# tub-rip/emba

Measured on AMD Instinct MI355X. Metric: events/sec through warp+Jacobian+JtJ build, 1M events, 1024x2048 pano, higher is better.
Workload: dtype f64; 1 GPU; synthetic N=1000000 sensor=240x180 pano=1024x2048 K=21 seed=20240907; events_per_gpu=1000000, total_events=1000000, thres_valid_pixel=5, cost=quadratic, parallelism=single GPU, events_per_rank=1000000, ep_in_step=True, inliers_rank0=675197, candidates_rank0=956800, active_pixels=68600

## Files before the change

emba_amd/csrc/context.h:

```cpp
#pragma once
#include "../../include/emba_hip.h"

#include <hip/hip_runtime.h>

#include <algorithm>
#include <cmath>
#include <cstdarg>
#include <cstdio>
#include <string>
#include <vector>

#include "kernels.h"
#include "solve_kernels.h"
#include "map_rule.h"
#include "cmax_rule.h"

struct DevBuf {
    void* p = nullptr;
    size_t bytes = 0;
    DevBuf() = default;
    DevBuf(DevBuf&& o) noexcept : p(o.p), bytes(o.bytes) { o.p = nullptr; o.bytes = 0; }
    DevBuf& operator=(DevBuf&& o) noexcept { if (this != &o) { reset(); std::swap(p, o.p); std::swap(bytes, o.bytes); } return *this; }
    ~DevBuf() { reset(); }
    template <typename T> T* as() const { return static_cast<T*>(p); }
// ... 94 lines not shown
    const uint8_t* global_u8 = nullptr;
    double fused_alpha = 0.0;
};

struct WindowState {
    bool have_events = false;
    size_t n_in = 0, n_used = 0, n_halo = 0, n_pm = 0, n_sorted = 0, n_batch = 0, n_cand = 0;
    long nblk = 0;
    long n_fblk = 0, n_fsup = 0;
    size_t P_prev = 0;
    size_t n_outside_tile = 0; int n_rebin = 0; uint32_t last_rebin_stamp = 0;
};

struct OrderState {
    bool keys_ready = false; int64_t key_t0 = 0, key_dt = 0; int key_K = 0;
    uint32_t* d_ev_pix = nullptr; uint32_t* d_ev_batch = nullptr;
    bool tile_order = false, have_ev_pm = false;
    long n_chunks = 0;
    size_t n_lead = 0;
    bool chunks_lpt = false;
    int tile_shape = 0; bool tile_fine = false;
    double order_per_px = 0.0, order_lead_frac = 0.0;
    double order_inl_pred = 0.0;
};

enum StatusWord : int {
    kStFirstBad = 0,
    kStUnsorted = 1,
    kStProbeA = 0, kStProbeB = 1,
    kStBadHalo = 2,
    kStTotal = 4,
    kStHeads = 6,
    kStCounter = 8,
    kStatusWords = 16
};

struct ListsKey {
    bool packed = false; uint32_t stamp = 0; size_t P = 0, nrec = 0; long lo = 0;
    bool operator==(const ListsKey& o) const { return packed == o.packed && stamp == o.stamp && P == o.P && nrec == o.nrec && lo == o.lo; }
};

struct SolveCache {
    bool lists_valid = false; ListsKey key;
    bool perm_valid = false;
    size_t perm_lo = 0, perm_n = 0;
    size_t x2_resident_P = (size_t)-1;
// ... 56 lines not shown
    bool spun = false;
    int* h_pinned_dev = nullptr;
    double* h_knots_dev = nullptr;

    WindowState win;
    OrderState order;
    DevBuf d_pm_pix, d_pm_batch, d_pm_orig;
    DevBuf d_ev_slot;
    DevBuf d_ev_pix_own, d_ev_batch_own;
    DevBuf d_ev_pm;
    DevBuf d_cp, d_batch_u;
    DevBuf d_ev_u, d_ev_seg;
    DevBuf d_chunks;
    int segpose_mode = 0;
    int order_mode = 0;
    DevBuf d_batch_t, d_pose;
    DevBuf d_seg;
    int step_gather = 2;
    DevBuf d_seg_act;
    PostWarpState post;
    int step_one_set = 1;
    int step_fast = 1;
    int use_tags = 1;
    DevBuf d_slot_key; uint32_t rec_stamp = 0;
    RecordSet work, alt;
    bool eq_in_alt = false;
    EqState eq, eq_saved;
    EvalState ev;
    DevBuf d_e_sorted, d_flag, d_inl_idx;
    int opt_poison = 0;
    int opt_tile_reserve = 2, opt_tile_shape = -1, opt_tile_fine = -1, opt_tile_min_events = 1650000, opt_tile_chunk = 0;
    int opt_gather_waves = 0, opt_chunk_order_bin = 0, opt_solve_counts = -1, opt_syrk_dense = 0, opt_syrk_lists = 0, opt_gram_sparse = -1, opt_gram_sparse_chunk = 4, opt_syrk_min_cols = 512, opt_syrk_item_cap = 4096, opt_solve_debug = 0, opt_poisson = 0, opt_gemm64 = 0;
    int step_ep = 1;
    DevBuf d_fblk_cnt, d_fblk_off;
    DevBuf d_fsup;
    DevBuf d_ep;
    double set_events_ms = 0, prepare_ms = 0;

    size_t n_inliers = 0;
    int cost_irls = 0; double cost_eta = 0.0;
    double* h_knots = nullptr; int h_knots_cap = 0; hipEvent_t knots_copied = nullptr; bool knots_in_flight = false;

    hipEvent_t ev_start[8]{}, ev_stop[8]{};
    bool kernel_timing = false;
    hipEvent_t kt_sets[16][5]{}; hipEvent_t* kt = kt_sets[0]; int kt_slot = 0;
    bool kt_valid[16][3]{};
    bool kt_all = false;
    hipEvent_t cal_ev[2]{};
    DevBuf d_probe;
    bool kt_warp_valid = false, kt_accum_valid = false;
    int n_cu = 256;
    int ablate = 0;
    struct {
        DevBuf scan_sums, scan_offs;
        DevBuf sort_hist;
// ... 87 lines not shown
```

emba_amd/csrc/emba_hip.hip:

```cpp
#include "../../include/emba_hip.h"

#include <hip/hip_runtime.h>

#include <algorithm>
#include <atomic>
#include <cmath>
#include <cstdarg>
#include <cstdio>
#include <cstdlib>
#include <cstring>
#include <limits>
#include <string>
#include <vector>

#include "kernels.h"
#include "order_kernels.h"
#include "solve_kernels.h"
#include "poisson_kernels.h"
#include "render_kernels.h"
#include "sequence_kernels.h"
#include "context.h"
#include "sequence_rule.h"

using namespace emba;
// ... 457 lines not shown
    {"tile_reserve", &emba_ctx::opt_tile_reserve, 0, 5},
    {"tile_shape", &emba_ctx::opt_tile_shape, -1, kNumTileShapes - 1},
    {"tile_fine", &emba_ctx::opt_tile_fine, -1, 1},
    {"tile_min_events", &emba_ctx::opt_tile_min_events, 0, 2000000000},
    {"tile_chunk", &emba_ctx::opt_tile_chunk, 0, 1 << 20},
    {"solve_counts", &emba_ctx::opt_solve_counts, -1, 2},
    {"syrk_dense", &emba_ctx::opt_syrk_dense, 0, 1},
    {"syrk_lists", &emba_ctx::opt_syrk_lists, 0, 2},
    {"gram_sparse", &emba_ctx::opt_gram_sparse, -1, 1},
    {"gram_sparse_chunk", &emba_ctx::opt_gram_sparse_chunk, 1, 8},
    {"syrk_min_cols", &emba_ctx::opt_syrk_min_cols, 64, 4096},
    {"syrk_item_cap", &emba_ctx::opt_syrk_item_cap, 1, 65536},
    {"solve_debug", &emba_ctx::opt_solve_debug, 0, 1},
    {"poisson", &emba_ctx::opt_poisson, 0, 2},
    {"gemm64", &emba_ctx::opt_gemm64, 0, 1},
};
const OptionRef kStepPrepOptions[] = {
    {"step_prep", &emba_ctx::step_prep, 0, 1},
    {"step_prep_polls", &emba_ctx::step_prep_polls, 0, 1 << 16},
};
const OptionRef kContrastOptions[] = {
    {"contrast_vote", &emba_ctx::opt_contrast_vote, -1, 1},
};
}

emba_status emba_set_option(emba_ctx* c, const char* name, int32_t value)
{
    if (!c || !name) return EMBA_ERR_INVALID_ARG;
    for (const OptionRef& o : kOptions)
        if (!strcmp(o.name, name)) {
            if (value < o.lo || value > o.hi) return fail(c, EMBA_ERR_INVALID_ARG, "option %s: %d outside [%d, %d]", name, (int)value, o.lo, o.hi);
            c->*(o.field) = (int)value;
            if (!strcmp(name, "order") || !strcmp(name, "chunk_order_bin") || !strncmp(name, "tile_", 5)) c->order.keys_ready = false;
            return EMBA_OK;
        }
    for (const OptionRef& o : kStepPrepOptions)
        if (!strcmp(o.name, name)) {
            if (value < o.lo || value > o.hi) return fail(c, EMBA_ERR_INVALID_ARG, "option %s: %d outside [%d, %d]", name, (int)value, o.lo, o.hi);
            c->*(o.field) = (int)value;
            return EMBA_OK;
        }
    for (const OptionRef& o : kContrastOptions)
        if (!strcmp(o.name, name)) {
            if (value < o.lo || value > o.hi) return fail(c, EMBA_ERR_INVALID_ARG, "option %s: %d outside [%d, %d]", name, (int)value, o.lo, o.hi);
            c->*(o.field) = (int)value;
            return EMBA_OK;
        }
    return fail(c, EMBA_ERR_INVALID_ARG, "unknown option '%s'", name);
}

emba_status emba_get_option(emba_ctx* c, const char* name, int32_t* value)
{
    if (!c || !name || !value) return EMBA_ERR_INVALID_ARG;
    if (!strcmp(name, "prep_in_warp")) { *value = c->ev.prep_in_warp ? 1 : 0; return EMBA_OK; }
    if (!strcmp(name, "texels_packed")) { *value = c->ev.texels_packed ? 1 : 0; return EMBA_OK; }
    if (!strcmp(name, "step_prep_fallbacks")) {
        unsigned n = 0;
        HIP_TRY(c, hipSetDevice(c->device));
        HIP_TRY(c, hipStreamSynchronize(c->stream));
        c->spun = false; c->knots_in_flight = false;
        HIP_TRY(c, hipMemcpy(&n, c->d_seg_flag.as<unsigned>() + 32, sizeof n, hipMemcpyDeviceToHost));
        *value = (int32_t)std::min<unsigned>(n, 0x7FFFFFFFu);
        return EMBA_OK;
    }
    if (!strcmp(name, "ep_valid")) { *value = c->ev.ep_valid ? 1 : 0; return EMBA_OK; }
    for (const OptionRef& o : kOptions)
        if (!strcmp(o.name, name)) { *value = c->*(o.field); return EMBA_OK; }
    for (const OptionRef& o : kStepPrepOptions)
        if (!strcmp(o.name, name)) { *value = c->*(o.field); return EMBA_OK; }
    if (!strcmp(name, "contrast_vote_path")) { *value = c->contrast_vote_path; return EMBA_OK; }
    for (const OptionRef& o : kContrastOptions)
        if (!strcmp(o.name, name)) { *value = c->*(o.field); return EMBA_OK; }
    return fail(c, EMBA_ERR_INVALID_ARG, "unknown option '%s'", name);
}

emba_status emba_last_counts(emba_ctx* c, size_t* n_inliers, size_t* P)
{
    if (!c) return EMBA_ERR_INVALID_ARG;
    HIP_TRY(c, hipSetDevice(c->device));
    emba_status st = resolve_pending(c, true);
    if (st) return st;
    if (n_inliers) *n_inliers = c->n_inliers;
    if (P) *P = c->eq.P;
    return EMBA_OK;
}

emba_status emba_sync(emba_ctx* c)
{
    if (!c) return EMBA_ERR_INVALID_ARG;
    HIP_TRY(c, hipSetDevice(c->device));
    emba_status st = resolve_pending(c);
    if (st) return st;
    HIP_TRY(c, hipStreamSynchronize(c->stream));
    c->spun = false;
// ... 352 lines not shown
```

emba_amd/csrc/kernels.h:

```cpp
#pragma once
#include <hip/hip_runtime.h>
#include <stdint.h>

#include "device_math.h"
#include "order_rule.h"
#include "step_rule.h"

#ifdef EMBA_DIAG
#define EMBA_ABL(word, bit) (((word) & (bit)) != 0)
#else
#define EMBA_ABL(word, bit) false
#endif

namespace emba {

constexpr uint32_t kNoSlot = 0xFFFFFFFFu;
constexpr uint32_t kInvalidPix = 0xFFFFFFFFu;

__device__ __forceinline__ bool record_valid(double tail_y, uint32_t stamp, uint32_t& pano_idx)
{
    pano_idx = (uint32_t)__double2loint(tail_y);
    return (uint32_t)__double2hiint(tail_y) == stamp && pano_idx != kInvalidPix;
}
__host__ __device__ __forceinline__ int32_t count_marker(uint32_t stamp) { return (int32_t)(0x80000000u | (stamp & 0x3FFFFFFFu)); }
// ... 1397 lines not shown
            const int i = b * 64 + threadIdx.x;
            if (p.seg) seg_thread(i, knots, p.K, p.seg);
            else pose_thread(i, p.batch_t_ns, p.nb, knots, p.K, p.t0_ns, p.dt_ns, p.pose, p.err);
        }
    } else if (b < p.n_pose + p.n_tex) {
        texel_rect_blocks((long)b - p.n_pose, p.n_tex, p.Gx, p.Gy, p.H, p.W, p.rect, p.texel);
    } else {
        prep_block(b - p.n_pose - p.n_tex, p.count, p.npix, p.pixacc);
    }
}

typedef double double4_t __attribute__((ext_vector_type(4)));

struct GramParams {
    const double* rec; const uint32_t* slot_key; long n_slots; int chunk;
    const uint32_t* active_bits; int irls; double eta;
    uint32_t stamp;
    const double* tag;
    double* A11; double* b1; int dim;
    int ablate;
    int gather_waves;
    int n_gram_blocks;
    const uint8_t* ep_flag; const double* ep_e; double* ep_out; const uint32_t* ep_fblk_cnt; long ep_n_pm, ep_n_fblk; const uint32_t* ep_fsup;
};

__device__ __forceinline__ void gram_atomic_out(double v, int row, int col, uint32_t key, double* A11, double* b1, int dim, int ablate)
{
    if (row >= 12 || v == 0.0 || EMBA_ABL(ablate, 32)) return;
    const int bc = 3 * (int)(key >> 16), bp = 3 * (int)(key & 0xFFFFu);
    const int grow = (row < 6) ? bc + row : bp + row - 6;
    if (col < 12) {
        const int gcol = (col < 6) ? bc + col : bp + col - 6;
        atomicAdd(A11 + (size_t)grow + (size_t)dim * gcol, v);
    } else if (col == 14) {
        atomicAdd(b1 + grow, v);
    }
}

typedef __attribute__((address_space(3))) uint32_t lds_u32_t;
typedef __attribute__((address_space(3))) double lds_f64_t;
__device__ __attribute__((noinline)) void gram_flush(double4_t ee, double4_t oe, double4_t oo, uint32_t key, double* A11, double* b1,
                                                     uint32_t dim_ablate, uint32_t lds_tag_tile)
{
    const int dim = (int)(dim_ablate & 0x3FFFFu), ablate = (int)(dim_ablate >> 18);
    uint32_t* const s_tag = (uint32_t*)(lds_u32_t*)(uintptr_t)((lds_tag_tile & 0xFFFFu) << 2);
    double* const s_tile = (double*)(lds_f64_t*)(uintptr_t)((lds_tag_tile >> 16) << 3);
// ... 39 lines not shown
            const int i = q + 4 * r;
            tile[(2 * i) * 16 + 2 * j] = e;
            tile[(2 * i + 1) * 16 + 2 * j] = x;
            tile[(2 * j) * 16 + 2 * i + 1] = x;
            tile[(2 * i + 1) * 16 + 2 * j + 1] = o;
        }
    }
}

__device__ __forceinline__ double rec_elem14(double2 v)
{
    return __hiloint2double(__builtin_amdgcn_ds_swizzle(__double2hiint(v.x), (7 << 5) | 0x18),
                            __builtin_amdgcn_ds_swizzle(__double2loint(v.x), (7 << 5) | 0x18));
}
__device__ __forceinline__ uint32_t rec_elem15_lo(double2 v)
{
    return (uint32_t)__builtin_amdgcn_ds_swizzle(__double2loint(v.y), (7 << 5) | 0x18);
}
__device__ __forceinline__ uint32_t rec_elem15_hi(double2 v)
{
    return (uint32_t)__builtin_amdgcn_ds_swizzle(__double2hiint(v.y), (7 << 5) | 0x18);
}

template <bool TAGS, int kGramBlock, bool GATHER, bool SPARSE = false>
__device__ __forceinline__ void gram_body(const GramParams& p, const long gram_blk, const ActiveWriteParams& aw)
{
    __shared__ uint32_t s_tag[kGramKeys];
    __shared__ double s_tile[kGramKeys * 256];
    __shared__ uint32_t s_pre[GATHER ? kGatherMaxUnits + 1 : 1];
    __shared__ uint32_t s_ws[kGramBlock / 64];
    __shared__ double s_wtile[(kGramBlock / 64) * 256];
    __shared__ uint32_t s_wkey[kGramBlock / 64];
    for (int i = threadIdx.x; i < kGramKeys * 256; i += kGramBlock) s_tile[i] = 0.0;
    if (threadIdx.x < kGramKeys) s_tag[threadIdx.x] = 0xFFFFFFFFu;
    if (threadIdx.x < kGramBlock / 64) s_wkey[threadIdx.x] = 0xFFFFFFFFu;
    const int kGW = GATHER ? __builtin_amdgcn_readfirstlane(p.gather_waves) : 0, kSW = kGramBlock / 64 - kGW;
    if (GATHER) {
        const uint32_t P_act = active_gather_prefix<kGramBlock>(aw, gram_blk, s_pre, s_ws);
        if (threadIdx.x < 64 * kGW) {
            if (kGW == 1) active_gather_slice<64>(aw, gram_blk, p.n_gram_blocks, P_act, s_pre);
            else if (kGW == 2) active_gather_slice<128>(aw, gram_blk, p.n_gram_blocks, P_act, s_pre);
            else active_gather_slice<256>(aw, gram_blk, p.n_gram_blocks, P_act, s_pre);
        }
    } else {
        __syncthreads();
    }
    const int lane = threadIdx.x & 63;
    const int wv = __builtin_amdgcn_readfirstlane(threadIdx.x >> 6) - kGW;
    constexpr int U = TAGS ? GRAM_U : GRAM_U_NT;
    constexpr int TS = GRAM_SPARSE_TS;
    constexpr int kStage = SPARSE ? 64 * TS : 8 * U;
    const int kStride = kSW * kStage;
    const long start = gram_blk * (kGramBlock / 64) * p.chunk;
    const long end = (start + (long)(kGramBlock / 64) * p.chunk < p.n_slots) ? start + (long)(kGramBlock / 64) * p.chunk : p.n_slots;
    const int len = (int)(end - start);
    const int off0 = wv * kStage;
    const bool have_work = wv >= 0 && off0 < len;
    const int m = lane & 7, R = lane >> 3;
    if (have_work) {

    uint32_t cur_key = p.slot_key[start + off0];
    bool dirty = false;
    double4_t acc_ee = {0.0, 0.0, 0.0, 0.0}, acc_oe = acc_ee, acc_oo = acc_ee;
    auto flush = [&]() {
        gram_flush(acc_ee, acc_oe, acc_oo, cur_key, p.A11, p.b1, (uint32_t)p.dim | ((uint32_t)p.ablate << 18),
                   (((uint32_t)(uintptr_t)(lds_u32_t*)s_tag >> 2) & 0xFFFFu) | (((uint32_t)(uintptr_t)(lds_f64_t*)s_tile >> 3) << 16));
#pragma unroll
        for (int r = 0; r < 4; ++r) { acc_ee[r] = 0.0; acc_oe[r] = 0.0; acc_oo[r] = 0.0; }
    };
    double2 xA[U], xB[U];
    uint32_t act[U], k_first = 0, k_last = 0;
    const double2* rec0 = reinterpret_cast<const double2*>(p.rec + (size_t)kRecStride * start) + lane;
    const uint32_t* key0 = p.slot_key + start;
    auto load_records = [&](int off, double2* x) {
        const double2* q = rec0 + 8 * off;
#pragma unroll
        for (int u = 0; u < U; ++u) {
            typedef double v2d __attribute__((ext_vector_type(2)));
            if (GRAM_NT_LOAD) { const v2d v = __builtin_nontemporal_load(reinterpret_cast<const v2d*>(q + 64 * u)); x[u] = make_double2(v.x, v.y); }
// ... 1 lines not shown
        }
    };
    auto lookup = [&](int off, const double2* x) {
        k_first = key0[off];
        k_last = key0[(off + 8 * U < len ? off + 8 * U : len) - 1];
#pragma unroll
        for (int u = 0; u < U; ++u) {
            const uint32_t pi = rec_elem15_lo(x[u]);
            const bool in = off + 8 * u + R < len;
            const bool valid = in && rec_elem15_hi(x[u]) == p.stamp && pi != kInvalidPix;
            act[u] = valid ? (EMBA_ABL(p.ablate, 256) ? ~0u : p.active_bits[pi >> 5]) >> (pi & 31) : 0u;
        }
    };
    auto weight = [&](const double2& x) {
        double w = 1.0;
        if (p.irls) {
            const double e = rec_elem14(x);
            if (p.irls == 2) w = 1.0 / (1.0 + p.eta * e * e);
            else { const double a = fabs(e); w = (a < p.eta) ? 1.0 : p.eta / a; }
        }
        return w;
    };
    auto consume = [&](int off, double2* x) {
        if ((k_first == cur_key) && (k_last == cur_key)) {
#pragma unroll
            for (int u = 0; u < U; ++u) {
                const bool ok = act[u] & 1u;
                const double w = weight(x[u]);
                const double ax = ok ? w * x[u].x : 0.0, ay = ok ? w * x[u].y : 0.0, bx = ok ? x[u].x : 0.0, by = ok ? x[u].y : 0.0;
                if (__ballot(ok)) {
                    dirty = true;
                    if (!EMBA_ABL(p.ablate, 64)) {
                        acc_ee = __builtin_amdgcn_mfma_f64_16x16x4f64(ax, bx, acc_ee, 0, 0, 0);
                        acc_oe = __builtin_amdgcn_mfma_f64_16x16x4f64(ay, bx, acc_oe, 0, 0, 0);
                        acc_oo = __builtin_amdgcn_mfma_f64_16x16x4f64(ay, by, acc_oo, 0, 0, 0);
                    }
                }
            }
            return;
        }
        double2* y = x;
        uint32_t* a_ = act;
#pragma unroll 1
        for (int u = 0; u < U; ++u) {
            const bool ok = a_[0] & 1u;
            const double w = weight(y[0]);
            const int s = off + 8 * u + R;
// ... 151 lines not shown
            const uint32_t bit = ((EMBA_ABL(p.ablate, 256) ? ~0u : w) >> ((uint32_t)__double2loint(tg) & 31u)) & (tagvalid(off, tg) ? 1u : 0u);
            return (unsigned long long)__ballot(bit != 0);
        };
        const double2* dummy = reinterpret_cast<const double2*>(p.rec + (size_t)kRecStride * start) + (lane & 7);
        auto load_masked = [&](int off, unsigned long long m, double2* x) {
            const double2* q = rec0 + 8 * off;
#pragma unroll
            for (int u = 0; u < U; ++u) {
#if GRAM_DUMMY_LOADS
                x[u] = *(((m >> (8 * u + R)) & 1u) ? q + 64 * u : dummy);
#else
                if (GRAM_TAG_NT) {
                    typedef double v2d __attribute__((ext_vector_type(2)));
                    v2d v = {0.0, 0.0};
                    if ((m >> (8 * u + R)) & 1u) v = __builtin_nontemporal_load(reinterpret_cast<const v2d*>(q + 64 * u));
                    x[u] = make_double2(v.x, v.y);
                } else
                x[u] = ((m >> (8 * u + R)) & 1u) ? q[64 * u] : make_double2(0.0, 0.0);
#endif
            }
        };
        typedef const uint32_t __attribute__((address_space(4))) * const_u32_ptr;
        const_u32_ptr key_s = (const_u32_ptr)(uintptr_t)key0;
        auto keys = [&](int off) { k_first = key_s[off]; k_last = key_s[(off + 8 * U < len ? off + 8 * U : len) - 1]; };
        static_assert(8 * U <= 64, "a stage's live mask is one wave ballot");
        unsigned long long Mc; uint32_t W;
        double Te, To;
        auto iterate = [&](int off, double2* cur, double2* nxt, double& Tb, double& Tn) {
            const bool h1 = off + kStride < len;
            const unsigned long long Mn = h1 ? bitmask(off + kStride, Tb, W) : 0ull;
            W = bitword(off + 2 * kStride, Tn);
            Tb = tagload(off + 3 * kStride);
            load_masked(h1 ? off + kStride : off, Mn, nxt);
            keys(off);
#pragma unroll
            for (int u = 0; u < U; ++u) act[u] = (Mc >> (8 * u + R)) & 1u;
            if (Mc) consume(off, cur);
            Mc = Mn;
        };
        Te = tagload(off0);
        W = bitword(off0, Te);
        To = tagload(off0 + kStride);
        Mc = bitmask(off0, Te, W);
        W = bitword(off0 + kStride, To);
        Te = tagload(off0 + 2 * kStride);
        load_masked(off0, Mc, xA);
        for (int off = off0; off < len;) {
// ... 37 lines not shown
    uint32_t actA[U];
    load_clamped(off0, xA);
    load_clamped(off0 + kStride, xB);
    load_clamped(off0 + 2 * kStride, xC);
    lookup_into(off0, xA, actA, kfA, klA);
    for (int off = off0; off < len;) {
        iterate(off, xA, xB, xD, actA, kfA, klA, actB, kfB, klB); off += kStride; if (off >= len) break;
        iterate(off, xB, xC, xA, actB, kfB, klB, actA, kfA, klA); off += kStride; if (off >= len) break;
        iterate(off, xC, xD, xB, actA, kfA, klA, actB, kfB, klB); off += kStride; if (off >= len) break;
        iterate(off, xD, xA, xC, actB, kfB, klB, actA, kfA, klA); off += kStride;
    }
    }
#if !GRAM_WAVE_TILE
    if (dirty) flush();
#else
    if (dirty) {
        const int wabs = threadIdx.x >> 6;
        gram_wave_tile(acc_ee, acc_oe, acc_oo, s_wtile + wabs * 256);
        if (lane == 0) s_wkey[wabs] = cur_key;
    }
#endif
    }
    __syncthreads();
    for (int i = threadIdx.x; i < kGramKeys * 256; i += kGramBlock) {
        const uint32_t key = s_tag[i >> 8];
        if (key != 0xFFFFFFFFu) gram_atomic_out(s_tile[i], (i >> 4) & 15, i & 15, key, p.A11, p.b1, p.dim, p.ablate);
    }
    if (threadIdx.x < 256) {
        const int e = threadIdx.x, row = e >> 4, col = e & 15;
        constexpr int NW = kGramBlock / 64;
        uint32_t kw[NW];
#pragma unroll
        for (int w = 0; w < NW; ++w) kw[w] = s_wkey[w];
        double tv[NW];
#pragma unroll
        for (int w = 0; w < NW; ++w) tv[w] = (kw[w] != 0xFFFFFFFFu) ? s_wtile[w * 256 + e] : 0.0;
        if (row < 12 && (col < 12 || col == 14)) {
#pragma unroll
            for (int w = 0; w < NW; ++w) {
                if (kw[w] == 0xFFFFFFFFu) continue;
                bool leader = true;
#pragma unroll
                for (int w2 = 0; w2 < w; ++w2) leader = leader && (kw[w2] != kw[w]);
                if (!leader) continue;
                double sum = 0.0;
#pragma unroll
// ... 26 lines not shown
        const double2 a = *reinterpret_cast<const double2*>(p.ep_e + i0), b = *reinterpret_cast<const double2*>(p.ep_e + i0 + 2);
        e[0] = a.x; e[1] = a.y; e[2] = b.x; e[3] = b.y;
    } else {
#pragma unroll
        for (int k = 0; k < 4; ++k) if (i0 + k < p.ep_n_pm) { fl |= (uint32_t)p.ep_flag[i0 + k] << (8 * k); e[k] = p.ep_e[i0 + k]; }
    }
    const uint32_t m = ((fl & 0xFFu) ? 1u : 0u) | ((fl & 0xFF00u) ? 2u : 0u) | ((fl & 0xFF0000u) ? 4u : 0u) | ((fl & 0xFF000000u) ? 8u : 0u);
    const uint32_t mine = __popc(m);
    uint32_t x = mine;
#pragma unroll
    for (int o = 1; o < 64; o <<= 1) { const uint32_t y = __shfl_up(x, o); if (lane >= o) x += y; }
#pragma unroll
    for (int o = 32; o >= 1; o >>= 1) part += __shfl_xor(part, o);
    if (lane == 63) s_x[wv] = x;
    if (lane == 0) s_b[wv] = part;
    __syncthreads();
    uint32_t k = x - mine;
#pragma unroll
    for (int w = 0; w < kGramBlock / 64; ++w) { k += s_b[w]; if (w < wv) k += s_x[w]; }
#pragma unroll
    for (int q = 0; q < 4; ++q) if (m & (1u << q)) p.ep_out[k++] = e[q];
}

template <bool TAGS, bool GATHER, bool SPARSE = false>
__global__ __launch_bounds__(kGramBlock) void emba_gram_kernel(GramParams p, ActiveWriteParams aw)
{
    if ((int)blockIdx.x >= p.n_gram_blocks) { ep_tail_block((long)blockIdx.x - p.n_gram_blocks, p); return; }
    gram_body<TAGS, kGramBlock, GATHER, SPARSE>(p, blockIdx.x, aw);
}

__global__ void emba_a22_from_records_kernel(const double* __restrict__ rec, long n_slots, const int32_t* __restrict__ count,
                                             const int32_t* __restrict__ compact, int thres, int irls, double eta,
                                             double* __restrict__ A22b2, uint32_t stamp)
{
    const long s = (long)blockIdx.x * blockDim.x + threadIdx.x;
    if (s >= n_slots) return;
    const double2* r2 = reinterpret_cast<const double2*>(rec + (size_t)kRecStride * s);
    const double2 tail = r2[7];
    uint32_t pi;
    if (!record_valid(tail.y, stamp, pi) || count[pi] < thres) return;
    const double e = tail.x;
    double w = 1.0;
    if (irls == 2) w = 1.0 / (1.0 + eta * e * e);
    else if (irls == 1) { const double a = fabs(e); w = (a < eta) ? 1.0 : eta / a; }
    const double ew = w * e;
    const double2 d = r2[6];
    double* q = A22b2 + 5 * (size_t)compact[pi];
    atomicAdd(q + 0, w * (d.x * d.x));
    atomicAdd(q + 1, w * (d.x * d.y));
    atomicAdd(q + 2, w * (d.y * d.y));
    atomicAdd(q + 3, d.x * ew);
// ... 206 lines not shown
```

emba_amd/csrc/order_host.h:

```cpp
#pragma once
#include "context.h"
#include "order_kernels.h"
#include "sequence_rule.h"

#include <chrono>

using namespace emba;

namespace {

OrderState new_order(const OrderState& prev)
{
    OrderState o{};
    o.tile_shape = prev.tile_shape; o.tile_fine = prev.tile_fine;
    return o;
}
void free_window(emba_ctx* c)
{
    WindowState w{};
    w.last_rebin_stamp = c->rec_stamp - 3;
    w.n_rebin = c->win.n_rebin;
    w.n_used = c->win.n_used; w.n_cand = c->win.n_cand; w.n_sorted = c->win.n_sorted; w.n_outside_tile = c->win.n_outside_tile;
    c->win = w;
    OrderState o = new_order(c->order);
// ... 254 lines not shown
emba_status assign_record_slots(emba_ctx* c, int K)
{
    hipStream_t s = c->stream;
    emba_status st;
    const size_t nd = c->win.n_sorted, M = c->win.n_cand;
    if ((st = ensure<uint32_t>(c, c->ord.pos, std::max<size_t>(nd, 1)))) return st;
    uint32_t *d_cf = c->ord.flags.as<uint32_t>(), *d_cpos = c->ord.pos.as<uint32_t>();
    if ((st = dev_scan(c, d_cf, d_cpos, nd, nullptr))) return st;
    if ((st = ensure_sort_pairs(c, std::max<size_t>(M, 1)))) return st;
    uint32_t *k0 = c->ord.keys[0].as<uint32_t>(), *v0 = c->ord.vals[0].as<uint32_t>(), *k1 = c->ord.keys[1].as<uint32_t>(), *v1 = c->ord.vals[1].as<uint32_t>();
    if ((st = ensure<uint32_t>(c, c->d_ev_slot, nd))) return st;
    HIP_TRY(c, hipMemsetAsync(c->d_ev_slot.as<uint32_t>(), 0xFF, std::max<size_t>(nd, 1) * 4, s));
    if (nd) hipLaunchKernelGGL(emba_cand_keys_kernel, dim3(nblocks(nd)), dim3(256), 0, s, c->order.d_ev_pix, c->order.d_ev_batch, c->d_cp.as<uint16_t>(), (long)nd, d_cpos, k0, v0);
    const int kb = bits_for((size_t)K);
    if (kb <= 8) {
        if (M) hipLaunchKernelGGL(emba_fold_keys_kernel, dim3(nblocks(M)), dim3(256), 0, s, k0, (long)M, 1);
        if ((st = dev_sort(c, &k0, &v0, &k1, &v1, M, 16))) return st;
        if (M) hipLaunchKernelGGL(emba_fold_keys_kernel, dim3(nblocks(M)), dim3(256), 0, s, k0, (long)M, 0);
    } else if ((st = dev_sort(c, &k0, &v0, &k1, &v1, M, 32))) return st;
    if (M) hipLaunchKernelGGL(emba_slot_assign_kernel, dim3(nblocks(M)), dim3(256), 0, s, k0, v0, (long)M, c->d_ev_slot.as<uint32_t>(), c->d_slot_key.as<uint32_t>());
    return EMBA_OK;
}

emba_status prepare_order(emba_ctx* c, const double* knots_host, int64_t t0, int64_t dt, int K)
{
    if (c->order.keys_ready && c->order.key_t0 == t0 && c->order.key_dt == dt && c->order.key_K == K) return EMBA_OK;
    if (dt <= 0 || K < 2 || K > 65535) return fail(c, EMBA_ERR_INVALID_ARG, "bad spline: dt_ns=%lld K=%d", (long long)dt, K);
    const auto t_begin = std::chrono::steady_clock::now();
    hipStream_t s = c->stream;
    emba_status st;
    const size_t ns = c->win.n_pm;
    c->order = new_order(c->order);
    TileOrderChoice choice;
    if ((st = order_batch_segments(c, t0, dt, K)) || (st = choose_tile_order(c, knots_host, t0, dt, K, &choice))) return st;
    if ((st = choice.tile ? build_tile_order(c, choice) : build_pixel_order(c))) return st;
    c->win.nblk = (long)((c->win.n_sorted + kWarpNew - 1) / kWarpNew);
    if ((st = assign_record_slots(c, K))) return st;
    if ((st = ensure<double>(c, c->d_e_sorted, ns)) || (st = ensure<uint8_t>(c, c->d_flag, ns)) || (st = ensure<int32_t>(c, c->d_inl_idx, ns))) return st;
    HIP_TRY(c, hipMemsetAsync(c->d_flag.as<uint8_t>(), 0, std::max<size_t>(ns, 1), s));
    HIP_TRY(c, hipGetLastError());
    HIP_TRY(c, hipStreamSynchronize(s));
    c->order.keys_ready = true; c->order.key_t0 = t0; c->order.key_dt = dt; c->order.key_K = K;
    c->prepare_ms = std::chrono::duration<double, std::milli>(std::chrono::steady_clock::now() - t_begin).count();
    return EMBA_OK;
}


emba_status size_record_set(emba_ctx* c, RecordSet& rs, size_t n_cand)
{
    bool rec_fresh = false, tag_fresh = false;
    emba_status st;
    if ((st = ensure<double>(c, rs.rec, (std::max<size_t>(n_cand, 1) + kGramPad) * kRecStride, &rec_fresh)) || (st = ensure<double>(c, rs.tag, n_cand + kGramPad, &tag_fresh)))
        return st;
    if (rec_fresh) HIP_TRY(c, hipMemsetAsync(rs.rec.p, 0, rs.rec.bytes, c->stream));
    if (tag_fresh) HIP_TRY(c, hipMemsetAsync(rs.tag.p, 0, rs.tag.bytes, c->stream));
    return EMBA_OK;
}

emba_status set_events_core(emba_ctx* c, const uint16_t* x, const uint16_t* y, const uint8_t* pol, const int64_t* t_dev, const int64_t* batch_t_host,
                            size_t n, const uint16_t* hx, const uint16_t* hy, const int64_t* hbt, size_t n_halo)
// ... 172 lines not shown
```

emba_amd/csrc/order_kernels.h:

```cpp
#pragma once
#include <hip/hip_runtime.h>
#include <stdint.h>

#include "device_math.h"
#include "order_rule.h"

namespace emba {

constexpr uint32_t kEvPol = 0x80000000u;
constexpr uint32_t kEvLead = 0x40000000u;
constexpr uint32_t kEvHasPred = 0x20000000u;
constexpr uint32_t kEvPixMask = 0x1FFFFFFFu;
constexpr uint32_t kValHalo = 0x80000000u;
constexpr uint32_t kNoBin = 0xFFFFFFFFu;

constexpr int kSortTile = 4096;
constexpr int kScanTile = 4096;

__global__ __launch_bounds__(256) void emba_scan_tile_sums_kernel(const uint32_t* __restrict__ in, long n, uint32_t* __restrict__ sums)
{
    __shared__ uint32_t s_w[4];
    const long base = (long)blockIdx.x * kScanTile + 16 * threadIdx.x;
    uint32_t acc = 0;
#pragma unroll
// ... 331 lines not shown
__global__ void emba_cand_flag_kernel(const uint32_t* __restrict__ ev_pix, long nd, uint32_t* __restrict__ cand_flag)
{
    const long j = (long)blockIdx.x * blockDim.x + threadIdx.x;
    if (j < nd) cand_flag[j] = (ev_pix[j] & kEvHasPred) ? 1u : 0u;
}

__global__ void emba_fold_keys_kernel(uint32_t* __restrict__ keys, long M, int fold)
{
    const long m = (long)blockIdx.x * blockDim.x + threadIdx.x;
    if (m >= M) return;
    const uint32_t k = keys[m];
    keys[m] = fold ? (((k >> 16) << 8) | (k & 0xFFu)) : (((k >> 8) << 16) | (k & 0xFFu));
}

__global__ void emba_slot_assign_kernel(const uint32_t* __restrict__ keys, const uint32_t* __restrict__ vals, long M, uint32_t* __restrict__ ev_slot,
                                        uint32_t* __restrict__ slot_key)
{
    const long s = (long)blockIdx.x * blockDim.x + threadIdx.x;
    if (s >= M) return;
    ev_slot[vals[s]] = (uint32_t)s;
    slot_key[s] = keys[s];
}

__global__ void emba_fill_u32_kernel(uint32_t* __restrict__ p, long n, uint32_t v)
{
    const long i = (long)blockIdx.x * blockDim.x + threadIdx.x;
    if (i < n) p[i] = v;
}

__global__ void emba_iota_kernel(uint32_t* __restrict__ p, long n)
{
    const long i = (long)blockIdx.x * blockDim.x + threadIdx.x;
    if (i < n) p[i] = (uint32_t)i;
}

__global__ __launch_bounds__(256) void emba_count_pred_inliers_kernel(const uint32_t* __restrict__ pm_pix, const uint32_t* __restrict__ pred, long ns, double outlier_px,
                                                                      unsigned long long* __restrict__ out)
{
    __shared__ uint32_t s_w[4];
    uint32_t acc = 0;
    const double lim2 = outlier_px * outlier_px;
    for (long i = (long)blockIdx.x * 256 + threadIdx.x; i < ns; i += (long)gridDim.x * 256) {
        if (i == 0 || !(pm_pix[i] & kEvHasPred) || (pm_pix[i] & kEvLead)) continue;
        const uint32_t a = pred[i], b = pred[i - 1];
        if (a == kNoPixel || b == kNoPixel) continue;
        const double dx = (double)(int)(a & 0xFFFFu) - (double)(int)(b & 0xFFFFu), dy = (double)(int)(a >> 16) - (double)(int)(b >> 16);
// ... 23 lines not shown
```

emba_amd/csrc/step_host.h:

```cpp
#pragma once
#include "context.h"
#include "step_rule.h"

using namespace emba;

namespace {

#define STEP_TRY(call) do { if (const emba_status st_ = (call)) return st_; } while (0)

constexpr GramSizes kGramSizes{kGramBlock, kGramChunk, kGramChunkMin, kEpTailBlk};

emba_status check_irls(emba_ctx* c, int32_t irls)
{
    if (irls < 0 || irls > 2) return fail(c, EMBA_ERR_INVALID_ARG, "irls must be 0 (quadratic), 1 (huber) or 2 (cauchy)");
    return EMBA_OK;
}

bool gram_uses_tags(const emba_ctx* c, bool ep_host) { return gram_tags(c->use_tags, c->order.tile_order, ep_host); }

emba_status ensure_pack(emba_ctx* c, int K)
{
    const PackLayout pack(K);
    if (c->pack_bound) {
        if (c->pack_cap < pack.head)
// ... 506 lines not shown
namespace {

emba_status override_ep(emba_ctx* c, const double* ep_host)
{
    hipStream_t s = c->stream;
    STEP_TRY(ensure_inl_idx(c));
    HIP_TRY(c, hipMemcpyAsync(c->d_ep.as<double>(), ep_host, c->n_inliers * sizeof(double), hipMemcpyHostToDevice, s));
    hipLaunchKernelGGL(emba_override_ep_kernel, dim3((unsigned)((c->win.n_sorted + 255) / 256)), dim3(256), 0, s, c->d_ep.as<double>(), c->d_flag.as<uint8_t>(),
                       c->d_inl_idx.as<int32_t>(), c->d_ev_slot.as<uint32_t>(), c->order.d_ev_pix, c->order.tile_order ? c->d_ev_pm.as<uint32_t>() : nullptr, (long)c->win.n_sorted, c->work.rec.as<double>(), c->d_e_sorted.as<double>());
    return EMBA_OK;
}

emba_status rebuild_a22_from_records(emba_ctx* c, int32_t irls, double eta)
{
    hipStream_t s = c->stream;
    STEP_TRY(ensure_compact(c));
    HIP_TRY(c, hipMemsetAsync(pack_A22b2(c), 0, 5 * c->eq.P * sizeof(double), s));
    if (c->win.n_cand)
        hipLaunchKernelGGL(emba_a22_from_records_kernel, dim3((unsigned)((c->win.n_cand + 255) / 256)), dim3(256), 0, s, c->work.rec.as<double>(),
                           (long)c->win.n_cand, c->d_count, c->d_compact.as<int32_t>(), c->eq.thres, irls, eta, pack_A22b2(c), c->work.stamp);
    return EMBA_OK;
}

void launch_gram_form(bool tags, bool gather, bool sparse, unsigned grid, hipStream_t s, const GramParams& p, const ActiveWriteParams& aw)
{
#define GRAM_FORM(...) hipLaunchKernelGGL((emba_gram_kernel<__VA_ARGS__>), dim3(grid), dim3(kGramBlock), 0, s, p, aw)
    if (tags && sparse) { if (gather) GRAM_FORM(true, true, true); else GRAM_FORM(true, false, true); }
    else if (tags) { if (gather) GRAM_FORM(true, true); else GRAM_FORM(true, false); }
    else { if (gather) GRAM_FORM(false, true); else GRAM_FORM(false, false); }
#undef GRAM_FORM
}

emba_status launch_gram(emba_ctx* c, bool ep_host, int32_t irls, double eta)
{
    hipStream_t s = c->stream;
    GramParams p{};
    p.rec = c->work.rec.as<double>(); p.slot_key = c->d_slot_key.as<uint32_t>(); p.n_slots = (long)c->win.n_cand;
    p.active_bits = reinterpret_cast<const uint32_t*>(c->d_active_bits.as<uint8_t>());
    p.irls = irls; p.eta = eta;
    p.stamp = c->work.stamp;
    p.A11 = pack_A11(c); p.b1 = pack_b1(c); p.dim = 3 * c->eq.K;
    p.tag = gram_uses_tags(c, ep_host) ? c->work.tag.as<double>() : nullptr;
    p.ablate = c->ablate;
    const bool sparse = gram_sparse(p.tag != nullptr, c->opt_gram_sparse, c->win.P_prev, c->win.n_cand, c->eq.thres);
    const bool ep_tail = c->ev.ep_in_gram && !ep_host && c->win.n_pm;
    const GramPlan plan = gram_plan(c->win.n_cand, sparse, c->opt_gram_sparse_chunk, c->n_cu, ep_tail, c->win.n_pm, c->opt_gather_waves, kGramSizes);
    p.chunk = plan.chunk;
    p.n_gram_blocks = plan.n_gram_blocks;
    p.gather_waves = plan.gather_waves;
    if (c->kernel_timing) HIP_TRY(c, hipEventRecord(c->kt[2], s));
    if (ep_tail) {
        p.ep_flag = c->d_flag.as<uint8_t>(); p.ep_e = c->d_e_sorted.as<double>(); p.ep_out = c->d_ep.as<double>();
        p.ep_fblk_cnt = c->d_fblk_cnt.as<uint32_t>(); p.ep_n_fblk = c->win.n_fblk;
        p.ep_n_pm = (long)c->win.n_pm;
        p.ep_fsup = c->d_fsup.as<uint32_t>() + (size_t)c->post.fsup_half * c->win.n_fsup * kFlagSupStride;
    }
    c->ev.ep_in_gram = false;
    const ActiveWriteParams aw = c->post.gather_deferred ? c->post.gather : ActiveWriteParams{};
    launch_gram_form(p.tag != nullptr, c->post.gather_deferred, sparse, plan.grid, s, p, aw);
    c->post.gather_deferred = false;
    if (ep_tail) c->ev.ep_valid = true;
    if (c->kernel_timing) { HIP_TRY(c, hipEventRecord(c->kt[3], s)); c->kt_accum_valid = true; c->kt_valid[c->kt_slot][1] = true; }
    return EMBA_OK;
}

emba_status launch_ep_after_gram(emba_ctx* c)
{
    STEP_TRY(dev_scan(c, c->d_fblk_cnt.as<uint32_t>(), c->d_fblk_off.as<uint32_t>(), (size_t)c->win.n_fblk, c->d_total.as<uint32_t>() + 2));
    hipLaunchKernelGGL(emba_compact_ep_kernel, dim3((unsigned)c->win.n_fblk), dim3(256), 0, c->stream, c->d_e_sorted.as<double>(), c->d_flag.as<uint8_t>(), (const uint32_t*)nullptr, c->d_fblk_off.as<uint32_t>(), (long)c->win.n_pm,
                       c->d_ep.as<double>(), (int32_t*)nullptr);
    c->ev.ep_valid = true;
    return EMBA_OK;
}

}

extern "C" emba_status emba_form_accumulate(emba_ctx* c, const double* ep_host, int32_t irls, double eta)
{
    if (!c) return EMBA_ERR_INVALID_ARG;
    if (!c->eq.active_done && !c->ev.P_pending) return fail(c, EMBA_ERR_STATE, "emba_form_active has not been called");
    if (c->eq.accum_done) return fail(c, EMBA_ERR_STATE, "these equations have been accumulated already: A11 | b1 are cleared by emba_form_active only (a second pass would add the sums again)");
    STEP_TRY(check_irls(c, irls));
// ... 131 lines not shown
```

emba_amd/csrc/step_rule.h:

```cpp
#pragma once
#include <stddef.h>
#include <stdint.h>

#include <algorithm>

#if defined(__HIPCC__)
#define EMBA_RULE_HD __host__ __device__
#else
#define EMBA_RULE_HD
#endif

namespace emba {

struct PackLayout {
    size_t b1, A22b2, head;
    explicit PackLayout(int K) : b1((size_t)9 * K * K), A22b2(b1 + (size_t)3 * K), head(A22b2) {}
    size_t len(size_t P) const { return head + 5 * P; }
    size_t need(size_t npix) const { return len(npix); }
    size_t max_P(size_t cap) const { return (cap - head) / 5; }
};

inline int hessian_source(int texel_mode, size_t n_sorted, size_t npix)
{
    return texel_mode == 1 ? 1 : texel_mode == 2 ? 0 : texel_mode == 3 ? 3 : (n_sorted > 4 * npix ? 1 : 3);
}

inline bool segpose_in_pixel_order(bool tile_order, int segpose_mode) { return !tile_order && (segpose_mode ? segpose_mode == 2 : true); }
// ... 46 lines not shown
struct GramPlan { int chunk; long waves; int n_gram_blocks; unsigned ep_tail_blocks, grid; int gather_waves; };
inline GramPlan gram_plan(size_t n_cand, bool sparse, int opt_gram_sparse_chunk, int n_cu, bool ep_tail, size_t n_pm, int opt_gather_waves, const GramSizes& k)
{
    GramPlan g{};
    const long chunk_cap = sparse ? (long)opt_gram_sparse_chunk * k.chunk : k.chunk;
    const long per_round = (long)n_cu * (k.block / 64);
    const long rounds = std::max<long>(1, ((long)n_cand + per_round * chunk_cap - 1) / (per_round * chunk_cap));
    long chunk = ((long)n_cand + per_round * rounds - 1) / (per_round * rounds);
    chunk = (chunk + 7) & ~7L;
    chunk = std::min<long>(std::max<long>(chunk, k.chunk_min), chunk_cap);
    g.chunk = (int)chunk;
    g.waves = ((long)n_cand + chunk - 1) / chunk;
    const long wpb = k.block / 64;
    g.grid = (unsigned)((g.waves + wpb - 1) / wpb);
    g.n_gram_blocks = (int)g.grid;
    if (ep_tail) {
        g.ep_tail_blocks = (unsigned)((n_pm + k.ep_tail_blk - 1) / k.ep_tail_blk);
        g.grid += g.ep_tail_blocks;
    }
    g.gather_waves = gather_waves(opt_gather_waves);
    return g;
}

inline bool tile_rebin_due(bool tile_order, size_t n_inliers, size_t n_outside_tile, uint32_t rec_stamp, uint32_t last_rebin_stamp)
{
    return tile_order && n_inliers && n_outside_tile * 5 > n_inliers && rec_stamp - last_rebin_stamp >= 3;
}

}
```

Measured before the change: 11.19 billion events/s.

## Align gram wave work ranges to single-key runs to skip shared tile merging

Adds a paired gram form. Each wave gets a precomputed [start,end) cut that lies inside one slot-key run, computed on the host from run starts collected after slot assignment. Because every stage then holds a single key, the kernel skips the per-stage key checks, the shared tile zeroing and the final tag-tile atomic flush. The cost is an extra kernel, a host sync and a copy at order preparation, plus possibly more waves and uneven load when runs are short.

```diff
diff --git a/emba_amd/csrc/context.h b/emba_amd/csrc/context.h
--- a/emba_amd/csrc/context.h
+++ b/emba_amd/csrc/context.h
@@ -140,6 +140,8 @@
     int tile_shape = 0; bool tile_fine = false;
     double order_per_px = 0.0, order_lead_frac = 0.0;
     double order_inl_pred = 0.0;
+    std::vector<uint32_t> run_start; bool runs_known = false;
+    int cuts_sw = 0, cuts_base_blocks = 0, cuts_blocks = 0;
 };
 
 enum StatusWord : int {
@@ -242,6 +244,7 @@
     int step_one_set = 1;
     int step_fast = 1;
     int use_tags = 1;
+    DevBuf d_gram_cuts; std::vector<uint32_t> h_gram_cuts; bool last_gram_paired = false;
     DevBuf d_slot_key; uint32_t rec_stamp = 0;
     RecordSet work, alt;
     bool eq_in_alt = false;
@@ -250,7 +253,7 @@
     DevBuf d_e_sorted, d_flag, d_inl_idx;
     int opt_poison = 0;
     int opt_tile_reserve = 2, opt_tile_shape = -1, opt_tile_fine = -1, opt_tile_min_events = 1650000, opt_tile_chunk = 0;
-    int opt_gather_waves = 0, opt_chunk_order_bin = 0, opt_solve_counts = -1, opt_syrk_dense = 0, opt_syrk_lists = 0, opt_gram_sparse = -1, opt_gram_sparse_chunk = 4, opt_syrk_min_cols = 512, opt_syrk_item_cap = 4096, opt_solve_debug = 0, opt_poisson = 0, opt_gemm64 = 0;
+    int opt_gather_waves = 0, opt_chunk_order_bin = 0, opt_solve_counts = -1, opt_syrk_dense = 0, opt_syrk_lists = 0, opt_gram_sparse = -1, opt_gram_sparse_chunk = 4, opt_gram_multikey = 0, opt_syrk_min_cols = 512, opt_syrk_item_cap = 4096, opt_solve_debug = 0, opt_poisson = 0, opt_gemm64 = 0;
     int step_ep = 1;
     DevBuf d_fblk_cnt, d_fblk_off;
     DevBuf d_fsup;
diff --git a/emba_amd/csrc/emba_hip.hip b/emba_amd/csrc/emba_hip.hip
--- a/emba_amd/csrc/emba_hip.hip
+++ b/emba_amd/csrc/emba_hip.hip
@@ -503,6 +503,9 @@
 const OptionRef kContrastOptions[] = {
     {"contrast_vote", &emba_ctx::opt_contrast_vote, -1, 1},
 };
+const OptionRef kGramOptions[] = {
+    {"gram_multikey", &emba_ctx::opt_gram_multikey, 0, 1},
+};
 }
 
 emba_status emba_set_option(emba_ctx* c, const char* name, int32_t value)
@@ -527,6 +530,12 @@
             c->*(o.field) = (int)value;
             return EMBA_OK;
         }
+    for (const OptionRef& o : kGramOptions)
+        if (!strcmp(o.name, name)) {
+            if (value < o.lo || value > o.hi) return fail(c, EMBA_ERR_INVALID_ARG, "option %s: %d outside [%d, %d]", name, (int)value, o.lo, o.hi);
+            c->*(o.field) = (int)value;
+            return EMBA_OK;
+        }
     return fail(c, EMBA_ERR_INVALID_ARG, "unknown option '%s'", name);
 }
 
@@ -551,6 +560,9 @@
         if (!strcmp(o.name, name)) { *value = c->*(o.field); return EMBA_OK; }
     if (!strcmp(name, "contrast_vote_path")) { *value = c->contrast_vote_path; return EMBA_OK; }
     for (const OptionRef& o : kContrastOptions)
+        if (!strcmp(o.name, name)) { *value = c->*(o.field); return EMBA_OK; }
+    if (!strcmp(name, "gram_paired")) { *value = c->last_gram_paired ? 1 : 0; return EMBA_OK; }
+    for (const OptionRef& o : kGramOptions)
         if (!strcmp(o.name, name)) { *value = c->*(o.field); return EMBA_OK; }
     return fail(c, EMBA_ERR_INVALID_ARG, "unknown option '%s'", name);
 }
diff --git a/emba_amd/csrc/kernels.h b/emba_amd/csrc/kernels.h
--- a/emba_amd/csrc/kernels.h
+++ b/emba_amd/csrc/kernels.h
@@ -1443,6 +1443,7 @@
     int gather_waves;
     int n_gram_blocks;
     const uint8_t* ep_flag; const double* ep_e; double* ep_out; const uint32_t* ep_fblk_cnt; long ep_n_pm, ep_n_fblk; const uint32_t* ep_fsup;
+    const uint32_t* wave_cuts;
 };
 
 __device__ __forceinline__ void gram_atomic_out(double v, int row, int col, uint32_t key, double* A11, double* b1, int dim, int ablate)
@@ -1528,7 +1529,7 @@
     return (uint32_t)__builtin_amdgcn_ds_swizzle(__double2hiint(v.y), (7 << 5) | 0x18);
 }
 
-template <bool TAGS, int kGramBlock, bool GATHER, bool SPARSE = false>
+template <bool TAGS, int kGramBlock, bool GATHER, bool SPARSE = false, bool PAIRED = false>
 __device__ __forceinline__ void gram_body(const GramParams& p, const long gram_blk, const ActiveWriteParams& aw)
 {
     __shared__ uint32_t s_tag[kGramKeys];
@@ -1537,8 +1538,11 @@
     __shared__ uint32_t s_ws[kGramBlock / 64];
     __shared__ double s_wtile[(kGramBlock / 64) * 256];
     __shared__ uint32_t s_wkey[kGramBlock / 64];
-    for (int i = threadIdx.x; i < kGramKeys * 256; i += kGramBlock) s_tile[i] = 0.0;
-    if (threadIdx.x < kGramKeys) s_tag[threadIdx.x] = 0xFFFFFFFFu;
+    static_assert(!PAIRED || (TAGS && !SPARSE && GRAM_WAVE_TILE), "the pair-aligned form is the dense tag-stream form with the waves' own tiles");
+    if constexpr (!PAIRED) {
+        for (int i = threadIdx.x; i < kGramKeys * 256; i += kGramBlock) s_tile[i] = 0.0;
+        if (threadIdx.x < kGramKeys) s_tag[threadIdx.x] = 0xFFFFFFFFu;
+    }
     if (threadIdx.x < kGramBlock / 64) s_wkey[threadIdx.x] = 0xFFFFFFFFu;
     const int kGW = GATHER ? __builtin_amdgcn_readfirstlane(p.gather_waves) : 0, kSW = kGramBlock / 64 - kGW;
     if (GATHER) {
@@ -1556,11 +1560,18 @@
     constexpr int U = TAGS ? GRAM_U : GRAM_U_NT;
     constexpr int TS = GRAM_SPARSE_TS;
     constexpr int kStage = SPARSE ? 64 * TS : 8 * U;
-    const int kStride = kSW * kStage;
-    const long start = gram_blk * (kGramBlock / 64) * p.chunk;
-    const long end = (start + (long)(kGramBlock / 64) * p.chunk < p.n_slots) ? start + (long)(kGramBlock / 64) * p.chunk : p.n_slots;
+    const int kStride = PAIRED ? kStage : kSW * kStage;
+    long start, end;
+    if constexpr (PAIRED) {
+        const uint32_t* cut = p.wave_cuts + 2 * (gram_blk * (kGramBlock / 64) + (wv > 0 ? wv : 0));
+        start = (long)__builtin_amdgcn_readfirstlane((int)cut[0]);
+        end = (long)__builtin_amdgcn_readfirstlane((int)cut[1]);
+    } else {
+        start = gram_blk * (kGramBlock / 64) * p.chunk;
+        end = (start + (long)(kGramBlock / 64) * p.chunk < p.n_slots) ? start + (long)(kGramBlock / 64) * p.chunk : p.n_slots;
+    }
     const int len = (int)(end - start);
-    const int off0 = wv * kStage;
+    const int off0 = PAIRED ? 0 : wv * kStage;
     const bool have_work = wv >= 0 && off0 < len;
     const int m = lane & 7, R = lane >> 3;
     if (have_work) {
@@ -1608,7 +1619,7 @@
         return w;
     };
     auto consume = [&](int off, double2* x) {
-        if ((k_first == cur_key) && (k_last == cur_key)) {
+        if (PAIRED || ((k_first == cur_key) && (k_last == cur_key))) {
 #pragma unroll
             for (int u = 0; u < U; ++u) {
                 const bool ok = act[u] & 1u;
@@ -1806,7 +1817,7 @@
         };
         typedef const uint32_t __attribute__((address_space(4))) * const_u32_ptr;
         const_u32_ptr key_s = (const_u32_ptr)(uintptr_t)key0;
-        auto keys = [&](int off) { k_first = key_s[off]; k_last = key_s[(off + 8 * U < len ? off + 8 * U : len) - 1]; };
+        auto keys = [&](int off) { if constexpr (!PAIRED) { k_first = key_s[off]; k_last = key_s[(off + 8 * U < len ? off + 8 * U : len) - 1]; } };
         static_assert(8 * U <= 64, "a stage's live mask is one wave ballot");
         unsigned long long Mc; uint32_t W;
         double Te, To;
@@ -1890,6 +1901,7 @@
 #endif
     }
     __syncthreads();
+    if constexpr (!PAIRED)
     for (int i = threadIdx.x; i < kGramKeys * 256; i += kGramBlock) {
         const uint32_t key = s_tag[i >> 8];
         if (key != 0xFFFFFFFFu) gram_atomic_out(s_tile[i], (i >> 4) & 15, i & 15, key, p.A11, p.b1, p.dim, p.ablate);
@@ -1962,11 +1974,11 @@
     for (int q = 0; q < 4; ++q) if (m & (1u << q)) p.ep_out[k++] = e[q];
 }
 
-template <bool TAGS, bool GATHER, bool SPARSE = false>
+template <bool TAGS, bool GATHER, bool SPARSE = false, bool PAIRED = false>
 __global__ __launch_bounds__(kGramBlock) void emba_gram_kernel(GramParams p, ActiveWriteParams aw)
 {
     if ((int)blockIdx.x >= p.n_gram_blocks) { ep_tail_block((long)blockIdx.x - p.n_gram_blocks, p); return; }
-    gram_body<TAGS, kGramBlock, GATHER, SPARSE>(p, blockIdx.x, aw);
+    gram_body<TAGS, kGramBlock, GATHER, SPARSE, PAIRED>(p, blockIdx.x, aw);
 }
 
 __global__ void emba_a22_from_records_kernel(const double* __restrict__ rec, long n_slots, const int32_t* __restrict__ count,
diff --git a/emba_amd/csrc/order_host.h b/emba_amd/csrc/order_host.h
--- a/emba_amd/csrc/order_host.h
+++ b/emba_amd/csrc/order_host.h
@@ -300,6 +300,28 @@
     return EMBA_OK;
 }
 
+emba_status collect_pair_runs(emba_ctx* c)
+{
+    hipStream_t s = c->stream;
+    const size_t M = c->win.n_cand;
+    c->order.run_start.clear(); c->order.runs_known = false;
+    if (!M) return EMBA_OK;
+    emba_status st;
+    if ((st = ensure<uint32_t>(c, c->ord.pos, 1 + (size_t)kGramMaxRuns))) return st;
+    uint32_t* d_runs = c->ord.pos.as<uint32_t>();
+    HIP_TRY(c, hipMemsetAsync(d_runs, 0, 4, s));
+    hipLaunchKernelGGL(emba_pair_runs_kernel, dim3(nblocks(M)), dim3(256), 0, s, c->d_slot_key.as<uint32_t>(), (long)M, d_runs, kGramMaxRuns);
+    uint32_t n = 0;
+    HIP_TRY(c, hipMemcpyAsync(&n, d_runs, 4, hipMemcpyDeviceToHost, s));
+    HIP_TRY(c, hipStreamSynchronize(s));
+    if (!n || n > kGramMaxRuns) return EMBA_OK;
+    c->order.run_start.resize(n);
+    HIP_TRY(c, hipMemcpy(c->order.run_start.data(), d_runs + 1, (size_t)n * 4, hipMemcpyDeviceToHost));
+    std::sort(c->order.run_start.begin(), c->order.run_start.end());
+    c->order.runs_known = true;
+    return EMBA_OK;
+}
+
 emba_status prepare_order(emba_ctx* c, const double* knots_host, int64_t t0, int64_t dt, int K)
 {
     if (c->order.keys_ready && c->order.key_t0 == t0 && c->order.key_dt == dt && c->order.key_K == K) return EMBA_OK;
@@ -313,7 +335,7 @@
     if ((st = order_batch_segments(c, t0, dt, K)) || (st = choose_tile_order(c, knots_host, t0, dt, K, &choice))) return st;
     if ((st = choice.tile ? build_tile_order(c, choice) : build_pixel_order(c))) return st;
     c->win.nblk = (long)((c->win.n_sorted + kWarpNew - 1) / kWarpNew);
-    if ((st = assign_record_slots(c, K))) return st;
+    if ((st = assign_record_slots(c, K)) || (st = collect_pair_runs(c))) return st;
     if ((st = ensure<double>(c, c->d_e_sorted, ns)) || (st = ensure<uint8_t>(c, c->d_flag, ns)) || (st = ensure<int32_t>(c, c->d_inl_idx, ns))) return st;
     HIP_TRY(c, hipMemsetAsync(c->d_flag.as<uint8_t>(), 0, std::max<size_t>(ns, 1), s));
     HIP_TRY(c, hipGetLastError());
diff --git a/emba_amd/csrc/order_kernels.h b/emba_amd/csrc/order_kernels.h
--- a/emba_amd/csrc/order_kernels.h
+++ b/emba_amd/csrc/order_kernels.h
@@ -377,6 +377,14 @@
     slot_key[s] = keys[s];
 }
 
+__global__ void emba_pair_runs_kernel(const uint32_t* __restrict__ slot_key, long M, uint32_t* __restrict__ out, uint32_t cap)
+{
+    const long s = (long)blockIdx.x * blockDim.x + threadIdx.x;
+    if (s >= M || (s && slot_key[s] == slot_key[s - 1])) return;
+    const uint32_t i = atomicAdd(out, 1u);
+    if (i < cap) out[1 + i] = (uint32_t)s;
+}
+
 __global__ void emba_fill_u32_kernel(uint32_t* __restrict__ p, long n, uint32_t v)
 {
     const long i = (long)blockIdx.x * blockDim.x + threadIdx.x;
diff --git a/emba_amd/csrc/step_host.h b/emba_amd/csrc/step_host.h
--- a/emba_amd/csrc/step_host.h
+++ b/emba_amd/csrc/step_host.h
@@ -552,13 +552,27 @@
     return EMBA_OK;
 }
 
-void launch_gram_form(bool tags, bool gather, bool sparse, unsigned grid, hipStream_t s, const GramParams& p, const ActiveWriteParams& aw)
+void launch_gram_form(bool tags, bool gather, bool sparse, bool paired, unsigned grid, hipStream_t s, const GramParams& p, const ActiveWriteParams& aw)
 {
 #define GRAM_FORM(...) hipLaunchKernelGGL((emba_gram_kernel<__VA_ARGS__>), dim3(grid), dim3(kGramBlock), 0, s, p, aw)
-    if (tags && sparse) { if (gather) GRAM_FORM(true, true, true); else GRAM_FORM(true, false, true); }
+    if (paired) { if (gather) GRAM_FORM(true, true, false, true); else GRAM_FORM(true, false, false, true); }
+    else if (tags && sparse) { if (gather) GRAM_FORM(true, true, true); else GRAM_FORM(true, false, true); }
     else if (tags) { if (gather) GRAM_FORM(true, true); else GRAM_FORM(true, false); }
     else { if (gather) GRAM_FORM(false, true); else GRAM_FORM(false, false); }
 #undef GRAM_FORM
+}
+
+emba_status ensure_gram_cuts(emba_ctx* c, int n_sw, const GramPlan& base)
+{
+    OrderState& o = c->order;
+    if (o.cuts_sw == n_sw && o.cuts_base_blocks == base.n_gram_blocks) return EMBA_OK;
+    const GramPairPlan g = gram_pair_cuts(o.run_start.data(), o.run_start.size(), c->win.n_cand, n_sw, base, kGramSizes, c->h_gram_cuts);
+    emba_status st;
+    if ((st = ensure<uint32_t>(c, c->d_gram_cuts, c->h_gram_cuts.size()))) return st;
+    HIP_TRY(c, hipStreamSynchronize(c->stream));
+    HIP_TRY(c, hipMemcpy(c->d_gram_cuts.as<uint32_t>(), c->h_gram_cuts.data(), c->h_gram_cuts.size() * sizeof(uint32_t), hipMemcpyHostToDevice));
+    o.cuts_sw = n_sw; o.cuts_base_blocks = base.n_gram_blocks; o.cuts_blocks = g.n_gram_blocks;
+    return EMBA_OK;
 }
 
 emba_status launch_gram(emba_ctx* c, bool ep_host, int32_t irls, double eta)
@@ -574,7 +588,15 @@
     p.ablate = c->ablate;
     const bool sparse = gram_sparse(p.tag != nullptr, c->opt_gram_sparse, c->win.P_prev, c->win.n_cand, c->eq.thres);
     const bool ep_tail = c->ev.ep_in_gram && !ep_host && c->win.n_pm;
-    const GramPlan plan = gram_plan(c->win.n_cand, sparse, c->opt_gram_sparse_chunk, c->n_cu, ep_tail, c->win.n_pm, c->opt_gather_waves, kGramSizes);
+    GramPlan plan = gram_plan(c->win.n_cand, sparse, c->opt_gram_sparse_chunk, c->n_cu, ep_tail, c->win.n_pm, c->opt_gather_waves, kGramSizes);
+    const bool paired = gram_paired(c->opt_gram_multikey, p.tag != nullptr, sparse, c->order.tile_order, c->order.runs_known, records_non_temporal(c->order.tile_order, c->win.n_cand, kRecStride));
+    if (paired) {
+        STEP_TRY(ensure_gram_cuts(c, kGramBlock / 64 - (c->post.gather_deferred ? plan.gather_waves : 0), plan));
+        p.wave_cuts = c->d_gram_cuts.as<uint32_t>();
+        plan.grid += (unsigned)(c->order.cuts_blocks - plan.n_gram_blocks);
+        plan.n_gram_blocks = c->order.cuts_blocks;
+    }
+    c->last_gram_paired = paired;
     p.chunk = plan.chunk;
     p.n_gram_blocks = plan.n_gram_blocks;
     p.gather_waves = plan.gather_waves;
@@ -587,7 +609,7 @@
     }
     c->ev.ep_in_gram = false;
     const ActiveWriteParams aw = c->post.gather_deferred ? c->post.gather : ActiveWriteParams{};
-    launch_gram_form(p.tag != nullptr, c->post.gather_deferred, sparse, plan.grid, s, p, aw);
+    launch_gram_form(p.tag != nullptr, c->post.gather_deferred, sparse, paired, plan.grid, s, p, aw);
     c->post.gather_deferred = false;
     if (ep_tail) c->ev.ep_valid = true;
     if (c->kernel_timing) { HIP_TRY(c, hipEventRecord(c->kt[3], s)); c->kt_accum_valid = true; c->kt_valid[c->kt_slot][1] = true; }
diff --git a/emba_amd/csrc/step_rule.h b/emba_amd/csrc/step_rule.h
--- a/emba_amd/csrc/step_rule.h
+++ b/emba_amd/csrc/step_rule.h
@@ -3,6 +3,7 @@
 #include <stdint.h>
 
 #include <algorithm>
+#include <vector>
 
 #if defined(__HIPCC__)
 #define EMBA_RULE_HD __host__ __device__
@@ -95,6 +96,40 @@
     return g;
 }
 
+constexpr uint32_t kGramMaxRuns = 4096;
+inline bool gram_paired(int opt_multikey, bool tags, bool sparse, bool tile_order, bool runs_known, bool records_nt)
+{
+    return !opt_multikey && tags && !sparse && !tile_order && runs_known && !records_nt;
+}
+struct GramPairPlan { int share; long waves; int n_gram_blocks; };
+inline GramPairPlan gram_pair_cuts(const uint32_t* run_start, size_t n_runs, size_t n_cand, int n_sw, const GramPlan& base, const GramSizes& k, std::vector<uint32_t>& cuts)
+{
+    const long wpb = k.block / 64;
+    const long slots = (long)base.n_gram_blocks * n_sw;
+    const long share_max = ((wpb * k.chunk + n_sw - 1) / n_sw + 7) & ~7L;
+    auto run_len = [&](size_t r) { return (long)((r + 1 < n_runs ? run_start[r + 1] : (uint32_t)n_cand) - run_start[r]); };
+    auto waves_at = [&](long share) { long n = 0; for (size_t r = 0; r < n_runs; ++r) n += (run_len(r) + share - 1) / share; return n; };
+    long share = (((long)n_cand + slots - 1) / std::max<long>(slots, 1) + 7) & ~7L;
+    share = std::min(std::max<long>(share, k.chunk_min), share_max);
+    while (share < share_max && waves_at(share) > slots) share += 8;
+    GramPairPlan g{};
+    g.share = (int)share;
+    g.waves = waves_at(share);
+    g.n_gram_blocks = (int)std::max<long>(1, (g.waves + n_sw - 1) / n_sw);
+    cuts.assign((size_t)g.n_gram_blocks * wpb * 2, 0u);
+    long w = 0;
+    for (size_t r = 0; r < n_runs; ++r) {
+        const long len = run_len(r), n = (len + share - 1) / share;
+        const long each = n ? (((len + n - 1) / n + 7) & ~7L) : 0;
+        for (long i = 0; i < n; ++i, ++w) {
+            const size_t at = (size_t)((w / n_sw) * wpb + w % n_sw) * 2;
+            cuts[at] = run_start[r] + (uint32_t)std::min(i * each, len);
+            cuts[at + 1] = run_start[r] + (uint32_t)std::min((i + 1) * each, len);
+        }
+    }
+    return g;
+}
+
 inline bool tile_rebin_due(bool tile_order, size_t n_inliers, size_t n_outside_tile, uint32_t rec_stamp, uint32_t last_rebin_stamp)
 {
     return tile_order && n_inliers && n_outside_tile * 5 > n_inliers && rec_stamp - last_rebin_stamp >= 3;
```

Result: faster. 11.60 billion events/s (median of 6 runs) (+3.7%).
